# TorchIO-project/torchio

Hardware: AMD Instinct MI355X
Metric: volumes/s (256^3 float32) for Compose[affine+elastic+bias+blur+noise] (higher is better)
Workload: dtype f32; 1 GPU; Compose[Affine(+-10deg,0.9-1.1,+-5mm),ElasticDeformation(7^3cp,7.5mm),BiasField,Blur(0.5-2mm),Noise] on 1x256^3 f32, per-instance params; batch_per_gpu=8, global_batch=8, noise_rng=philox, resample_precision=tight, stencil_precision=fast, parallelism=batch-split x1 (no data-path collective)

## Files before the change

### torchio_amd/csrc/api.hip

```cpp
#include <stdarg.h>
#include <stdio.h>
#include <stdlib.h>
#include <string.h>

#include <atomic>
#include <mutex>

#include "common.hpp"

namespace tio {

static thread_local char g_error[512] = "";

void set_error(const char* fmt, ...) {
  va_list ap;
  va_start(ap, fmt);
  vsnprintf(g_error, sizeof(g_error), fmt, ap);
  va_end(ap);
}

int fail(int status, const char* fmt, ...) {
  va_list ap;
  va_start(ap, fmt);
  vsnprintf(g_error, sizeof(g_error), fmt, ap);
  va_end(ap);
  return status;
}

int check_launch(const char* what) {
  const hipError_t err = hipGetLastError();
  if (err != hipSuccess) return fail(TIO_ERR_LAUNCH, "%s: launch failed: %s", what, hipGetErrorString(err));
  return TIO_OK;
}

static std::atomic<const EnvSwitches*> g_env{nullptr};
static std::mutex g_env_mu;

static const EnvSwitches* parse_env() {
  EnvSwitches* e = new EnvSwitches();
  auto num = [](const char* name, int unset) { const char* v = getenv(name); return v != nullptr ? atoi(v) : unset; };
  e->nearest_kernel = num("TIO_NEAREST_KERNEL", 1) != 0;
  if (const char* v = getenv("TIO_NEAREST_EPS")) { e->has_nearest_eps = 1; e->nearest_eps = static_cast<float>(atof(v)); }
  if (const char* v = getenv("TIO_RESAMPLE_PATH")) e->resample_path = strcmp(v, "gather") == 0 ? 1 : (strcmp(v, "tile") == 0 ? 2 : 0);
  e->tile_variant = num("TIO_TILE_VARIANT", 0);
  e->tile_lds_floats = num("TIO_TILE_LDS_FLOATS", 0);
  e->tile_ablate = num("TIO_TILE_ABLATE", 0);
  e->resample_exact = getenv("TIO_RESAMPLE_EXACT") != nullptr;
  if (const char* v = getenv("TIO_FAST_KERNEL")) e->fast_kernel = strcmp(v, "brick") == 0 ? 1 : (strcmp(v, "planned") == 0 ? 2 : 0);
  e->planned_lean = num("TIO_PLANNED_LEAN", 1) != 0;
  e->dma_packed = num("TIO_DMA_PACKED", 1) != 0;
  e->exact_plan = num("TIO_EXACT_PLAN", -1);
  e->exact_lean = num("TIO_EXACT_LEAN", -1);
  e->lean_interleave = num("TIO_LEAN_INTERLEAVE", 1);
  e->lean_multi = num("TIO_LEAN_MULTI", 1);
  e->nearest_exact = num("TIO_NEAREST_EXACT", 1);
  e->lean_pair = num("TIO_LEAN_PAIR", 1);
  e->lean_label = num("TIO_LEAN_LABEL", 1);
  e->nearest_lds = num("TIO_NEAREST_LDS", -1);
  e->fast_fill_recheck = num("TIO_FAST_FILL_RECHECK", 1) != 0;
  e->conv_no_fuse = getenv("TIO_CONV_NO_FUSE") != nullptr;
  e->conv_ring = getenv("TIO_CONV_RING") != nullptr;
  e->march_segs = num("TIO_MARCH_SEGS", 0);
  e->march_order = num("TIO_MARCH_ORDER", -1);
  e->min_blocks = num("TIO_MIN_BLOCKS", 0);
  return e;
}

const EnvSwitches& env_switches() {
  const EnvSwitches* e = g_env.load(std::memory_order_acquire);
  if (e != nullptr) return *e;
  std::lock_guard<std::mutex> lock(g_env_mu);
  e = g_env.load(std::memory_order_acquire);
  if (e == nullptr) { e = parse_env(); g_env.store(e, std::memory_order_release); }
  return *e;
}

}

extern "C" void tio_reload_env(void) {
  std::lock_guard<std::mutex> lock(tio::g_env_mu);
  tio::g_env.store(tio::parse_env(), std::memory_order_release);
}

extern "C" int tio_abi_version(void) { return TIO_ABI_VERSION; }

extern "C" const char* tio_last_error(void) { return tio::g_error; }
// ... 10 lines not shown
```

### torchio_amd/csrc/common.hpp

```cpp
#pragma once

#include <hip/hip_runtime.h>
#include <stdint.h>

#include "../../include/tio_hip.h"

namespace tio {

void set_error(const char* fmt, ...);
int fail(int status, const char* fmt, ...);
int check_launch(const char* what);

struct EnvSwitches {
  int nearest_kernel = 1;
  int has_nearest_eps = 0;
  float nearest_eps = 0.0f;
  int resample_path = 0;
  int tile_variant = 0;
  int tile_lds_floats = 0;
  int tile_ablate = 0;
  int resample_exact = 0;
  int fast_kernel = 0;
  int planned_lean = 1;
  int dma_packed = 1;
  int exact_plan = -1;
  int exact_lean = -1;
  int nearest_exact = 1;
  int nearest_lds = -1;
  int lean_pair = 1;
  int lean_label = 1;
  int lean_multi = 1;
  int lean_interleave = 1;
  int fast_fill_recheck = 1;
  int conv_no_fuse = 0;
  int conv_ring = 0;
  int march_segs = 0;
  int march_order = -1;
  int min_blocks = 0;
};
const EnvSwitches& env_switches();

__device__ __forceinline__ float bf16_bits_to_float(uint16_t h) {
  return __uint_as_float(static_cast<uint32_t>(h) << 16);
}

__device__ __forceinline__ uint16_t float_to_bf16_bits(float f) {
  uint32_t x = __float_as_uint(f);
  if ((x & 0x7FFFFFFFu) > 0x7F800000u) return 0x7FC0u;
  x += 0x7FFFu + ((x >> 16) & 1u);
  return static_cast<uint16_t>(x >> 16);
}

template <int DT>
struct Elem;
template <>
struct Elem<TIO_F32> {
  using type = float;
  static __device__ __forceinline__ float load(const void* p, int64_t i) { return static_cast<const float*>(p)[i]; }
  static __device__ __forceinline__ void store(void* p, int64_t i, float v) { static_cast<float*>(p)[i] = v; }
};
template <>
struct Elem<TIO_F64> {
  using type = double;
  static __device__ __forceinline__ float load(const void* p, int64_t i) {
// ... 141 lines not shown
```

### torchio_amd/csrc/resample.hip

```cpp
#include <type_traits>
#include <stdlib.h>
#include <string.h>

#include <mutex>
#include <vector>
#include <algorithm>

#include "common.hpp"

namespace tio {

struct ImgArgs {
  const void* in;
  void* out;
  const float* fill;
  int channels;
  int dtype;
  int interp;
  const double* labels;
  int n_labels;
  double pad_label;
  float* out_min;
  uint32_t* min_keys;
};
// ... 780 lines not shown
    if (s.interp == TIO_LABEL_PV) {
      if (s.channels != 1)
        return fail(TIO_ERR_INVALID_ARGUMENT, "tio_resample3d: image %d: TIO_LABEL_PV needs channels == 1, got %d", i, s.channels);
      if (s.n_labels < 0 || (s.n_labels > 0 && s.labels_dev == nullptr))
        return fail(TIO_ERR_INVALID_ARGUMENT, "tio_resample3d: image %d: bad label table", i);
      pv.img[pv.n_images++] = ImgArgs{s.in, s.out, nullptr, 1, s.dtype, s.interp, s.labels_dev, s.n_labels, s.pad_label, nullptr, nullptr};
      continue;
    }
    if (nn_enabled && s.interp == TIO_NEAREST && s.out_min_dev == nullptr) {
      nn.img[nn.n_images++] = NearestImg{s.in, s.out, s.channels, dtype_size(s.dtype), s.fill_dev, s.dtype};
      if (s.fill_dev != nullptr) nn.any_fill = 1;
      continue;
    }
    a.img[a.n_images++] = ImgArgs{s.in, s.out, s.fill_dev, s.channels, s.dtype, s.interp, nullptr, 0, 0.0, s.out_min_dev, nullptr};
    if (s.interp == TIO_LINEAR || s.interp == TIO_LINEAR_ADJOINT || s.fill_dev != nullptr) a.any_linear = 1;
    if (s.interp == TIO_NEAREST) a.any_nearest = 1;
    const int need = s.dtype == TIO_F32 ? 0 : ((s.dtype == TIO_I16 || s.dtype == TIO_U8 || s.dtype == TIO_I32) ? 1 : 2);
    group.dtmode = need > group.dtmode ? need : group.dtmode;
    group.rows16 = group.rows16 && (reinterpret_cast<uintptr_t>(s.in) & 15) == 0;
  }
  return TIO_OK;
}

enum FloatRoadKind { kRoadGather, kRoadBrick, kRoadPlannedBrick, kRoadFastBrick, kRoadPlannedFast, kRoadPlannedLean, kRoadLeanExact };

struct FloatRoad {
  FloatRoadKind kind = kRoadGather;
  int variant = 0;
  bool exact_lerp = false;
  int64_t bricks = 0;
  size_t lds = 0;
  size_t plan_need = 0;
  int cp_lds = 0, tile_cap = 0, ablate = 0, fill_recheck = 0, dma_packed = 0, plan_multi = 0;
  int interleave = 0, pair = 0;
};
FloatRoad choose_float_road(const tio_resample_geom& geom, const ResampleArgs& a, const FloatGroup& g, const EnvSwitches& env) {
  FloatRoad r;
  bool use_tile = a.any_linear != 0;
  if (env.resample_path == 1) use_tile = false;
  if (env.resample_path == 2) use_tile = true;
  if (g.any_adjoint) use_tile = false;
  if (static_cast<int64_t>(a.Jo) * a.Ko * 8 >= (1LL << 31)) use_tile = false;
  if (static_cast<int64_t>(a.I) * a.J * a.K >= (1LL << 30)) use_tile = false;
  if (!use_tile) return r;
  r.kind = kRoadBrick;
  r.variant = env.tile_variant;
  r.ablate = env.tile_ablate;
  r.fill_recheck = env.fast_fill_recheck;
  r.cp_lds = control_points_fit_lds(a) ? ((control_floats(a) + 3) & ~3) : 0;
  const int bpc = r.variant == 3 ? 2 : ((r.variant == 2 || r.variant == 4) ? 4 : kTileBlocksPerCU);
  const int cap = env.tile_lds_floats > 0 ? env.tile_lds_floats : kLdsFloatsPerCU / bpc - 512 - r.cp_lds - kTileRedInts;
  const int max_cap = kLdsFloatsPerCU - r.cp_lds - kTileRedInts;
  r.tile_cap = cap < kTileMinCap ? kTileMinCap : (cap > max_cap ? max_cap : cap);
  r.lds = static_cast<size_t>(r.cp_lds + kTileRedInts + r.tile_cap) * sizeof(float);
  r.bricks = static_cast<int64_t>(a.B) * ((a.Io + 15) / 16) * ((a.Jo + 15) / 16) * ((a.Ko + 15) / 16);
  const size_t plan_plain = static_cast<size_t>(a.B) * 16 + static_cast<size_t>(r.bricks) * kDescInts;
  const bool fast = geom.precision == TIO_PRECISION_FAST && g.dtmode == 0 && !a.any_nearest && r.variant == 0 && !env.resample_exact;
  const bool tight = geom.precision == TIO_PRECISION_TIGHT && !env.resample_exact;
  const bool lean_exact = !fast && (tight || ((geom.precision == TIO_PRECISION_EXACT || geom.precision == TIO_PRECISION_TIGHT) && env.exact_lean != 0)) &&
                          g.dtmode == 0 && !a.any_nearest && r.variant == 0 && r.ablate == 0 && a.short_div != 0 && (a.cp == nullptr || a.unit_spacing != 0);
  if (fast || lean_exact) {
    const bool force_planned = lean_exact ? (env.fast_kernel == 2 || env.exact_lean == 2) : env.fast_kernel == 2;
    bool planned = (lean_exact || env.fast_kernel != 1) && (a.K & 3) == 0 && (r.bricks >= kPlannedMinBricks || force_planned) && r.bricks < (1LL << 26) && g.rows16;
    if ((geom.flags & (TIO_GEOM_LARGE_BOXES | TIO_GEOM_MOSTLY_LARGE_BOXES)) != 0 && !force_planned && !lean_exact) planned = false;
    if (planned && a.cp != nullptr) {
      const int n_ctl[3] = {a.ni, a.nj, a.nk}, n_vox[3] = {a.Io, a.Jo, a.Ko};
      for (int d = 0; d < 3; d++)
        if (n_ctl[d] > 2 && (n_vox[d] - 1) < 16 * (n_ctl[d] - 1)) planned = false;
    }
    if (planned) {
      r.kind = lean_exact ? kRoadLeanExact : (env.planned_lean != 0 ? kRoadPlannedLean : kRoadPlannedFast);
      r.exact_lerp = !tight;
      const int cap_p = env.tile_lds_floats > 0 ? env.tile_lds_floats : (kLdsFloatsPerCU / kTileBlocksPerCU) / 320 * 320;
      r.tile_cap = cap_p < kTileMinCap ? kTileMinCap : (cap_p > kLdsFloatsPerCU ? kLdsFloatsPerCU : cap_p);
      r.cp_lds = 0;
      r.lds = static_cast<size_t>(r.tile_cap) * sizeof(float);
      r.dma_packed = env.dma_packed;
      r.interleave = env.lean_interleave;
      r.pair = env.lean_pair;
      if (lean_exact && env.lean_multi != 0)
        r.plan_multi = (geom.flags & TIO_GEOM_MOSTLY_LARGE_BOXES) != 0 ? 2 : ((geom.flags & TIO_GEOM_LARGE_BOXES) != 0 ? 1 : 0);
      const size_t n = static_cast<size_t>(r.bricks);
      const size_t plan_multi_ints = static_cast<size_t>(a.B) * 16 + n * (kDescInts + kPassInts * kPassesPerBrick) + ((n + 3) & ~static_cast<size_t>(3));
      r.plan_need = (kPlanHeaderInts + (r.plan_multi ? plan_multi_ints : plan_plain)) * sizeof(int);
      return r;
    }
    if (fast) {
      r.kind = kRoadFastBrick;
      return r;
    }
  }
  if (r.variant == 0 && r.ablate == 0 && a.cp == nullptr && env.exact_plan != 0 && (r.bricks >= kPlannedMinBricks || env.exact_plan == 2) && r.bricks < (1LL << 26)) {
    r.kind = kRoadPlannedBrick;
    r.plan_need = (kPlanHeaderInts + plan_plain) * sizeof(int);
  }
  return r;
}

void apply_road(ResampleArgs& a, const FloatRoad& r) {
  a.fill_recheck = r.fill_recheck; a.ablate = r.ablate; a.cp_lds = r.cp_lds; a.tile_cap = r.tile_cap;
  a.dma_packed = r.dma_packed; a.plan_multi = r.plan_multi;
  for (int i = 0; i < a.n_images && r.kind != kRoadGather; i++) a.any_fill |= a.img[i].fill != nullptr ? 1 : 0;
}

LeanArgs make_lean_args(const ResampleArgs& a, const FloatRoad& r, const int* plan, int n_items) {
  LeanArgs la{};
  la.plan = plan; la.cp = a.cp;
  la.I = a.I; la.J = a.J; la.K = a.K; la.Io = a.Io; la.Jo = a.Jo; la.Ko = a.Ko;
  la.B = a.B; la.n_items = n_items;
  la.bricks_per_element = static_cast<unsigned>(a.tiles_i) * a.tiles_j * a.tiles_k;
  la.bpe_magic = magic_u32(la.bricks_per_element);
  la.ni = a.ni; la.nj = a.nj; la.nk = a.nk; la.cp_batched = a.cp_batched;
  la.sci = a.scale_i; la.scj = a.scale_j; la.sck = a.scale_k;
  for (int e = 0; e < 3; e++) la.dsc[e] = a.rsp[e] * (a.affine_first ? a.half_h[e] / a.dh[e] : 1.0f);
  la.hx = a.size_m1[0]; la.hy = a.size_m1[1]; la.hz = a.size_m1[2];
  la.affine_first = a.affine_first; la.ablate = a.ablate;
  la.mapping = a.mapping; la.mapping_batched = a.mapping_batched; la.unit_spacing = a.unit_spacing; la.fill_recheck = a.fill_recheck;
  for (int e = 0; e < 3; e++) { la.sp[e] = a.sp[e]; la.rsp[e] = a.rsp[e]; la.den[e] = a.den[e]; la.rden[e] = a.rden[e]; }
  for (int e = 0; e < 3; e++) { la.dh[e] = a.dh[e]; la.rdh[e] = a.rdh[e]; la.half_h[e] = a.half_h[e]; }
  la.interleave = r.interleave;
  la.tile_floats = r.tile_cap;
  return la;
}

struct LabelRide {
  int es = 0;
  unsigned blocks = 0, lds = 0;
};
void launch_nearest_exact(const NearestArgs& nn, int es, unsigned blocks, unsigned lds, hipStream_t s) {
  with_element_size(es, [&](auto size) {
    with_bools([&](auto elastic) { hipLaunchKernelGGL((resample_nearest_exact_kernel<elastic.value, size.value>), dim3(blocks), dim3(256), lds, s, nn); }, nn.cp != nullptr);
  });
}

int launch_nearest(NearestArgs& nn, bool short_div, bool floats_alone, const EnvSwitches& env, hipStream_t s, LabelRide* label) {
  const bool rows = nn.Ko >= 48;
  unsigned blocks = 0;
  if (const int st = set_tiles(nn, 16, rows ? 4 : 16, rows ? 64 : 16, &blocks)) return st;
  nn.eps = env.has_nearest_eps ? env.nearest_eps : kNearestEps;
  const bool exact = env.nearest_exact != 0 && nn.any_fill == 0 && rows && short_div && (nn.cp == nullptr || nn.unit_spacing != 0);
  const unsigned exact_lds = env.nearest_lds >= 0 ? static_cast<unsigned>(env.nearest_lds) : (nn.cp == nullptr ? 52000u : 0u);
  for (int es = 1; es <= 8; es *= 2) {
    bool present = false;
    for (int i = 0; i < nn.n_images; i++) present = present || nn.img[i].es == es;
    if (!present) continue;
    const int64_t n_in = static_cast<int64_t>(nn.I) * nn.J * nn.K, n_out = static_cast<int64_t>(nn.Io) * nn.Jo * nn.Ko;
    const bool narrow = static_cast<int64_t>(nn.I) * nn.J <= (1 << 24) && static_cast<int64_t>(nn.K) * es < (1 << 24) &&
                        n_in * es < (int64_t{1} << 32) - 16 && n_out * es < (int64_t{1} << 32) - 16;
    if (exact && narrow && env.lean_label != 0 && nn.n_images == 1 && nn.img[0].channels == 1 && es <= 4 && floats_alone) {
      label->es = es; label->blocks = blocks; label->lds = exact_lds;
    } else if (exact && narrow) {
      launch_nearest_exact(nn, es, blocks, exact_lds, s);
    } else {
// ... 257 lines not shown
```

### torchio_amd/csrc/resample_fast.hpp

```cpp
#pragma once

namespace tio {

typedef __attribute__((address_space(3))) const float* fast_lds_ptr;
typedef __attribute__((address_space(3))) float* fast_lds_wptr;

__device__ __forceinline__ void fast_axis(float src, int n, int& i0, int& i1, float& l) {
  const float c = fminf(fmaxf(floorf(src), 0.0f), static_cast<float>(n > 1 ? n - 2 : 0));
  i0 = static_cast<int>(c);
  i1 = min(i0 + 1, n - 1);
  l = fminf(fmaxf(src - c, 0.0f), 1.0f);
}

template <typename CP>
struct FastFrameT {
  float m[12];
  double c[3];
  int j_lo, k_lo;
  bool elastic, affine_first;
  CP cp;
  int ni, nj, nk;
  float sci, scj, sck;
  float dsc[3];
};
// ... 471 lines not shown
#pragma unroll
    for (int q = 0; q < 12; q++) {
      const float mv = m[q];
      weird |= (__float_as_uint(mv) & 0x7FFFFFFFu) > 0x7149F2CAu;
      f.m[q] = mv * ratio[q >> 2];
    }
  }
#pragma unroll
  for (int e = 0; e < 3; e++) f.dsc[e] = a.rsp[e] * (f.affine_first ? ratio[e] : 1.0f);
  if constexpr (ELASTIC_POSSIBLE) {
    f.elastic = !(a.cp_skip != nullptr && a.cp_skip[p.b] != 0);
    f.cp = f.elastic ? a.cp + (a.cp_batched ? static_cast<int64_t>(p.b) * (a.ni * a.nj * a.nk * 3) : 0) : nullptr;
  }
  pipe_brick_frame(f, p.j_lo, p.k_lo);
  int ext[7] = {-0x40000000, -0x40000000, -0x40000000, -0x40000000, -0x40000000, -0x40000000, 0};
  const int n_vert = f.elastic ? 27 : 8;
  if (v < n_vert) {
    int r[6]; bool bad;
    pipe_vertex(a, f, v, p.i_begin, p.i_count, p.nv, p.nw, r, bad);
#pragma unroll
    for (int q = 0; q < 6; q++) ext[q] = r[q];
    ext[6] = bad ? 1 : 0;
  }
#pragma unroll
  for (int s = GROUP / 2; s > 0; s >>= 1) {
#pragma unroll
    for (int q = 0; q < 7; q++) ext[q] = max(ext[q], __shfl_xor(ext[q], s));
  }
  const PlanBox whole = plan_box(a, ext, weird);
  const bool wrd = weird | (ext[6] != 0);
  int kind = whole.outside ? kDescOutside : (whole.fits ? kDescStaged : kDescSlow);
  PlanBox first = whole;
  int d15 = 0;
  if (a.plan_multi != 0 && kind == kDescSlow && !wrd) {
    int* passes = plan + a.B * 16 + n_items * kDescInts + t * (kPassInts * kPassesPerBrick);
    for (int nsplit = 2; nsplit <= 4; nsplit *= 2) {
      const int span = TI / nsplit;
      bool all_ok = true;
      for (int q = 0; q < nsplit; q++) {
        const int u0 = p.i_begin + q * span, n = min(span, p.i_begin + p.i_count - u0);
        int e7[7] = {-0x40000000, -0x40000000, -0x40000000, -0x40000000, -0x40000000, -0x40000000, 0};
        if (v < n_vert && n > 0) {
          int r[6]; bool bad;
          pipe_vertex(a, f, v, u0, n, p.nv, p.nw, r, bad);
#pragma unroll
          for (int c = 0; c < 6; c++) e7[c] = r[c];
          e7[6] = bad ? 1 : 0;
        }
#pragma unroll
        for (int sft = GROUP / 2; sft > 0; sft >>= 1) {
#pragma unroll
          for (int c = 0; c < 7; c++) e7[c] = max(e7[c], __shfl_xor(e7[c], sft));
        }
        PlanBox pb = plan_pass_box(a, e7, weird);
        if (n <= 0) { pb.outside = 1; pb.fits = 0; pb.interior = 0; }
        all_ok &= (pb.fits | pb.outside) != 0;
        const int state = pb.outside ? kPassOutside : (pb.fits ? kPassStaged : kPassSlow);
        if (q == 0) { first = pb; d15 = nsplit; }
        d15 |= state << (8 + 4 * q);
        if (v == 0) {
          int* r8 = passes + q * kPassInts;
          r8[0] = pb.xmin; r8[1] = pb.ymin; r8[2] = pb.za; r8[3] = pb.Lx; r8[4] = pb.Ly; r8[5] = pb.cpr;
          r8[6] = state | (pb.interior << 8); r8[7] = max(n, 0);
        }
      }
      kind = kDescMulti;
// ... 181 lines not shown
        first = false;
      }
      float A3[3], B3[3];
      int run0 = u0;
      int run1 = fast_column_line(f, lj, lk, planes, run0, u1, u0, C3, col3, lane, A3, B3);
      tile_dma_wait();
      __syncthreads();
      const bool track = g.out_min != nullptr && b == 0;
      uint32_t kmin = 0xFFFFFFFFu;
      unsigned unsure = 0u;
      const float margin = (a.fill_recheck != 0 && has_fill) ? ((const_float_ptr)(plan) + b * 16)[12] : -1.0f;
      if (col_active) {
        for (;;) {
          char* o_run = out_chan + static_cast<int64_t>(run0) * slab_b;
          if (track)
            fast_sample_line<4, true>(run1 - run0, A3, B3, ta, o_run, urow, slab_b, has_fill & !bx.interior, ox, oy, oz, hx, hy, hz, fillv, kmin, margin, run0 - u0, unsure);
          else
            fast_sample_line<4, false>(run1 - run0, A3, B3, ta, o_run, urow, slab_b, has_fill & !bx.interior, ox, oy, oz, hx, hy, hz, fillv, kmin, margin, run0 - u0, unsure);
          run0 = run1;
          if (run0 >= u1) break;
          run1 = fast_column_line(f, lj, lk, planes, run0, u1, u0, C3, col3, lane, A3, B3);
        }
      }
      if (has_fill & !bx.interior)
        fast_fill_tail<ELASTIC_POSSIBLE>(unsure, a, a.mapping + (a.mapping_batched ? b * 12 : 0), elastic, f.cp, lj, lk, u0, static_cast<float>(j_lo + jv),
                                         static_cast<float>(k_lo + kw), in_chan, a.I, a.J, a.K, hx, hy, hz, fillv, out_chan, slab_b, urow, track ? &kmin : nullptr);
      if (track) publish_min(g, c, kmin);
    }
  }
}



struct LeanArgs {
  const float* in;
  float* out;
  int64_t in_stride, out_stride;
  const float* fill;
  const int* plan;
  const float* cp;
  int I, J, K, Io, Jo, Ko;
  int B, n_items;
  unsigned bricks_per_element, bpe_magic;
  int ni, nj, nk, cp_batched;
  float sci, scj, sck;
  float dsc[3];
  float hx, hy, hz;
  int affine_first, ablate;
  const float* mapping;
  int mapping_batched, unit_spacing, fill_recheck;
  float sp[3], rsp[3], den[3], rden[3];
  float dh[3], rdh[3], half_h[3];
  int interleave;
  int tile_floats;
  int last_use;
  uint32_t* min_keys;
  const float* in2;
  float* out2;
  int64_t in_stride2, out_stride2;
  const float* fill2;
  const void* lab_in;
  void* lab_out;
  int lab_es;
};

__device__ __forceinline__ float lean_gather(const float* __restrict__ chan, int I, int J, int K, float x, float y, float z, bool has_fill,
// ... 221 lines not shown
```

### torchio_amd/csrc/resample_lean_exact.hpp

```cpp
#pragma once

namespace tio {

__device__ __forceinline__ void tile_dma_wait_all() { asm volatile("s_waitcnt vmcnt(0) lgkmcnt(0)" ::: "memory"); }

template <int NW>
struct BoxDmaStepper {
  typedef __attribute__((address_space(1))) const char* global_byte_ptr;
  global_byte_ptr origin;
  float* lp;
  unsigned off, step_b, wrap_b;
  int row, p, r;
  int step, step_p, step_r, total_rows, Ly, lp_step;
  int bx0, by0, I, J;
  int left;
  bool ch_ok, lane_ok;

  __device__ __forceinline__ void init(float* tile, const float* src, const StreamBox& bx, int I_, int J_, int K, int wave, int lane) {
    StageLanes sl;
    sl.cpr = -1; sl.rpi = 1; sl.row_l = 0; sl.gz_rel = 0; sl.goff = 0; sl.lane_ok = false;
    stage_lanes(sl, bx.cpr, K, lane);
    const int rpi = sl.rpi;
    total_rows = bx.Lx * bx.Ly;
    const int n_instr = __builtin_amdgcn_readfirstlane(static_cast<int>((static_cast<float>(total_rows + rpi - 1) + 0.5f) * __builtin_amdgcn_rcpf(static_cast<float>(rpi))));
    step = NW * rpi;
    const float rcp_ly = __builtin_amdgcn_rcpf(static_cast<float>(bx.Ly));
    step_p = __builtin_amdgcn_readfirstlane(static_cast<int>((static_cast<float>(step) + 0.5f) * rcp_ly));
    step_r = step - step_p * bx.Ly;
    row = wave * rpi + sl.row_l;
    p = static_cast<int>((static_cast<float>(row) + 0.5f) * rcp_ly);
    r = row - p * bx.Ly;
    const unsigned plane_b = static_cast<unsigned>(J_) * static_cast<unsigned>(K) * 4u, row_b = static_cast<unsigned>(K) * 4u;
    off = static_cast<unsigned>(p) * plane_b + static_cast<unsigned>(r) * row_b + static_cast<unsigned>(sl.gz_rel) * 4u;
    step_b = static_cast<unsigned>(step_p) * plane_b + static_cast<unsigned>(step_r) * row_b;
    wrap_b = plane_b - static_cast<unsigned>(bx.Ly) * row_b;
    origin = (global_byte_ptr)(src) + ((static_cast<int64_t>(bx.bx0) * J_ + bx.by0) * K + bx.za) * 4;
    const int dgroup = rpi * bx.cpr * 4;
    lp = tile + wave * dgroup;
    lp_step = NW * dgroup;
    ch_ok = static_cast<unsigned>(bx.za + sl.gz_rel) < static_cast<unsigned>(K);
    lane_ok = sl.lane_ok;
    Ly = bx.Ly; bx0 = bx.bx0; by0 = bx.by0; I = I_; J = J_;
    left = n_instr > wave ? (n_instr - wave + NW - 1) / NW : 0;
  }

  template <bool INTERIOR>
  __device__ __forceinline__ void issue(int lane) {
    const bool in_box = lane_ok & (row < total_rows);
    if constexpr (INTERIOR) {
      if (in_box) __builtin_amdgcn_global_load_lds(origin + off, (fast_lds_wptr)(lp), 16, 0, 0);
    } else {
      const bool in_vol = in_box & ch_ok & (static_cast<unsigned>(bx0 + p) < static_cast<unsigned>(I)) &
                          (static_cast<unsigned>(by0 + r) < static_cast<unsigned>(J));
      if (in_vol) __builtin_amdgcn_global_load_lds(origin + off, (fast_lds_wptr)(lp), 16, 0, 0);
      else if (in_box) {
        lds_zero_chunk(lp + 4 * lane);
      }
    }
    row += step; p += step_p; r += step_r; off += step_b;
    if (r >= Ly) { r -= Ly; p += 1; off += wrap_b; }
    lp += lp_step;
    left -= 1;
  }
};

template <int MODE, bool UNIT, bool SHORT>
__device__ __forceinline__ void lean_exact_coord(const float (&m)[12], const LeanArgs& a, float ci, float cj, float ck, float di, float dj,
                                                 float dk, float& x, float& y, float& z) {
#define TIO_LE_ROW(R, A, B, C) \
  __builtin_fmaf(1.0f, m[4 * R + 3], __builtin_fmaf(C, m[4 * R + 2], __builtin_fmaf(B, m[4 * R + 1], __fmul_rn(A, m[4 * R]))))
  float vi, vj, vk;
  if constexpr (MODE == 0) {
    vi = TIO_LE_ROW(0, ci, cj, ck); vj = TIO_LE_ROW(1, ci, cj, ck); vk = TIO_LE_ROW(2, ci, cj, ck);
  } else {
    float qi = di, qj = dj, qk = dk;
    if constexpr (!UNIT) {
// ... 127 lines not shown
  const bool by0 = (y0 >= 0.0f) & (y0 <= hy), by1 = (y1 >= 0.0f) & (y1 <= hy);
  const bool bz0 = (z0 >= 0.0f) & (z0 <= hz), bz1 = (z1 >= 0.0f) & (z1 <= hz);
  const int ix0 = static_cast<int>(fminf(fmaxf(x0, 0.0f), hx)), ix1 = static_cast<int>(fminf(fmaxf(x1, 0.0f), hx));
  const int iy0 = static_cast<int>(fminf(fmaxf(y0, 0.0f), hy)), iy1 = static_cast<int>(fminf(fmaxf(y1, 0.0f), hy));
  const int iz0 = static_cast<int>(fminf(fmaxf(z0, 0.0f), hz)), iz1 = static_cast<int>(fminf(fmaxf(z1, 0.0f), hz));
  float val = 0.0f, mask = 0.0f;
#pragma unroll
  for (int k = 0; k < 8; k++) {
    const float w = __fmul_rn(__fmul_rn((k & 1) ? wx1 : wx0, (k & 2) ? wy1 : wy0), (k & 4) ? wz1 : wz0);
    const bool ok = ((k & 1) ? bx1 : bx0) & ((k & 2) ? by1 : by0) & ((k & 4) ? bz1 : bz0);
    const int off = (((k & 1) ? ix1 : ix0) * J + ((k & 2) ? iy1 : iy0)) * K + ((k & 4) ? iz1 : iz0);
    const float v = chan[off];
    const float next_v = __fadd_rn(val, __fmul_rn(v, w));
    const float next_m = __fadd_rn(mask, w);
    val = ok ? next_v : val;
    mask = ok ? next_m : mask;
  }
  if (has_fill) val = (mask > 0.5f) ? val : fillv;
  return val;
}

template <bool EXACT_LERP, bool MASKED>
__device__ __forceinline__ void lean_exact_group_values(const float (&X4)[4], const float (&Y4)[4], const float (&Z4)[4], const TileAddr& ta, float hx,
                                                        float hy, float hz, bool has_fill, float fillv, float (&vals)[4]) {
  TapSet ts[4];
#pragma unroll
  for (int u = 0; u < 4; u++) tile_issue_folded(ts[u], X4[u], Y4[u], Z4[u], ta);
  __builtin_amdgcn_sched_barrier(0);
#pragma unroll
  for (int u = 0; u < 4; u++) {
    float val = EXACT_LERP ? tile_finish(ts[u]) : tile_finish_fast(ts[u]);
    if constexpr (MASKED) val = (!has_fill || tile_mask(ts[u], X4[u], Y4[u], Z4[u], hx, hy, hz) > 0.5f) ? val : fillv;
    vals[u] = val;
  }
}

template <bool GUARD, bool TRACK>
__device__ __forceinline__ void lean_exact_group_store(const float (&vals)[4], char*& out_generic, unsigned urow, int64_t slab_b, int t0, int i_count,
                                                       bool col_active, uint32_t& kmin) {
  typedef __attribute__((address_space(1))) char* global_char_ptr;
  typedef __attribute__((address_space(1))) float* global_float_ptr;
  global_char_ptr out_t = (global_char_ptr)out_generic;
  unsigned row_off = urow;
  asm volatile("" : "+v"(row_off));
#pragma unroll
  for (int u = 0; u < 4; u++) {
    const bool live = !GUARD || (col_active && (t0 + u) < i_count);
    if (live) {
      *(global_float_ptr)(out_t + row_off) = vals[u];
      if constexpr (TRACK) kmin = min(kmin, float_to_key(vals[u]));
    }
    out_t += slab_b;
    asm volatile("" : "+s"(out_t));
  }
  out_generic = (char*)out_t;
}

template <bool EXACT_LERP, bool MASKED, bool GUARD, bool TRACK>
__device__ __forceinline__ void lean_exact_group(const float (&X4)[4], const float (&Y4)[4], const float (&Z4)[4], const TileAddr& ta, char*& out_generic,
                                                 unsigned urow, int64_t slab_b, int t0, int i_count, bool col_active, float hx, float hy,
                                                 float hz, bool has_fill, float fillv, uint32_t& kmin) {
  float vals[4];
  lean_exact_group_values<EXACT_LERP, MASKED>(X4, Y4, Z4, ta, hx, hy, hz, has_fill, fillv, vals);
  lean_exact_group_store<GUARD, TRACK>(vals, out_generic, urow, slab_b, t0, i_count, col_active, kmin);
  __builtin_amdgcn_sched_barrier(0);
}
// ... 164 lines not shown
  if (ka->ablate & 512) return;
  if (es == 1) TIO_LE_LABEL_STORES(uint8_t)
  else if (es == 2) TIO_LE_LABEL_STORES(uint16_t)
  else TIO_LE_LABEL_STORES(uint32_t)
#undef TIO_LE_LABEL_STORES
}

template <bool ELASTIC_POSSIBLE, bool EXACT_LERP, bool FOLD_MIN, bool MULTI, bool PAIR = false, bool LABEL = false>
__device__ __forceinline__ void lean_exact_brick(const LeanArgs& a, const unsigned brick, float* s_tile) {
  static_assert(!PAIR || (!FOLD_MIN && !MULTI), "the pair kernel has no folded minimum and no passes");
  static_assert(!LABEL || (!FOLD_MIN && !MULTI), "a label channel rides along launches without a folded minimum and without passes");
  constexpr int TI = 16, TJ = 16, TK = 16, NW = 4;
  typedef __attribute__((address_space(4))) const int* const_int_ptr;
  typedef __attribute__((address_space(4))) const float* const_float_ptr;

  {
    const int* plan_p = a.plan; const float* in_p = a.in; const float* map_p = a.mapping; float* out_p = a.out; const float* fill_p = a.fill;
    asm volatile("" ::"s"(a.n_items), "s"(a.bricks_per_element), "s"(a.bpe_magic), "s"(plan_p), "s"(in_p), "s"(map_p), "s"(a.B), "s"(a.I), "s"(a.J), "s"(a.K),
                 "s"(a.mapping_batched), "s"(a.tile_floats), "s"(a.in_stride), "s"(a.out_stride), "s"(a.Io), "s"(a.Jo), "s"(a.Ko), "s"(a.interleave),
                 "s"(out_p), "s"(fill_p), "s"(a.hx), "s"(a.hy), "s"(a.hz), "s"(a.affine_first));
    if constexpr (ELASTIC_POSSIBLE) {
      const float* cp_p = a.cp;
      asm volatile("" ::"s"(cp_p), "s"(a.cp_batched), "s"(a.ni), "s"(a.nj), "s"(a.nk), "s"(a.sci), "s"(a.scj), "s"(a.sck));
    }
  }
  const int b = static_cast<int>(fastdiv_exact(brick, a.bpe_magic, a.bricks_per_element));
  const_int_ptr d = (const_int_ptr)(a.plan + a.B * 16) + static_cast<size_t>(brick) * kDescInts;
  const_float_ptr mp = (const_float_ptr)(a.mapping) + (a.mapping_batched ? b * 12 : 0);
  const int kind_w = d[0];
  StreamBox bx;
  bx.bx0 = d[1]; bx.by0 = d[2]; bx.za = d[3]; bx.Lx = d[4]; bx.Ly = d[5]; bx.cpr = d[6];
  const int i_begin = d[11], j_lo = d[12], k_lo = d[13];
  const int elastic_w = d[14];
  int multi_w = 0, plan_tile = 0;
  if constexpr (MULTI) {
    multi_w = d[15];
    plan_tile = ((const_int_ptr)(a.plan))[b * 16 + 13];
  }
  float m[12];
#pragma unroll
  for (int q = 0; q < 12; q++) m[q] = mp[q];
  asm volatile("" ::"s"(kind_w), "s"(i_begin), "s"(j_lo), "s"(k_lo), "s"(elastic_w));
  if constexpr (MULTI) asm volatile("" ::"s"(multi_w), "s"(plan_tile));
  const bool elastic = ELASTIC_POSSIBLE && elastic_w != 0;

  const int tid = threadIdx.x;
  const int lane = tid & 63;
  const int wave = __builtin_amdgcn_readfirstlane(tid >> 6);
  const int tk = tid & (TK - 1), tj = tid / TK;
  const int slab = a.Jo * a.Ko;
  const int64_t slab_b = static_cast<int64_t>(slab) * 4;
  const float* in_chan = a.in + static_cast<int64_t>(b) * a.in_stride;
  char* out_chan = reinterpret_cast<char*>(a.out + static_cast<int64_t>(b) * a.out_stride);

  int kind = kind_w & 0xFF;
  const bool multi = MULTI && kind == kDescMulti;
  if constexpr (!MULTI) {
    if (kind == kDescMulti) return;
  }
  int nsplit = 1, states = 0;
  if constexpr (MULTI) {
    if (multi) {
      nsplit = multi_w & 0xF; states = multi_w >> 8;
      kind = plan_tile <= a.tile_floats ? kDescStaged : kDescSlow;
    }
  }
  if (!multi && kind == kDescStaged && (static_cast<int64_t>(bx.Lx) * bx.Ly * (bx.cpr * 4) > static_cast<int64_t>(a.tile_floats) ||
                                        !box_address_fits(bx.bx0, bx.by0, bx.za, bx.Lx, bx.Ly, bx.cpr)))
    kind = kDescSlow;
  if (kind == kDescSlow) states = 0x2222;
  const int span_shift = nsplit == 4 ? 2 : (nsplit == 2 ? 3 : 4);
  bx.kind = kind; bx.interior = kind_w >> 8;
  BoxDmaStepper<NW> dma;
  dma.left = 0;
  if (kind == kDescStaged && (states & 0xF) == kPassStaged) dma.init(s_tile, in_chan, bx, a.I, a.J, a.K, wave, lane);

  const int i_count = min(TI, a.Io - i_begin), nv = min(TJ, a.Jo - j_lo), nw = min(TK, a.Ko - k_lo);
  const bool col_active = (tj < nv) & (tk < nw);
  const bool full = (i_count == TI) & (nv == TJ) & (nw == TK);
  const int jv = min(tj, nv - 1), kw = min(tk, nw - 1);
  const int col_off = (j_lo + jv) * a.Ko + (k_lo + kw);
  const unsigned urow = static_cast<unsigned>(col_off) * 4u;
  bool has_fill = a.fill != nullptr;
  float fillv = has_fill ? ((const_float_ptr)a.fill)[0] : 0.0f;
  const float hx = a.hx, hy = a.hy, hz = a.hz;

  const bool track = FOLD_MIN && a.min_keys != nullptr && b == 0;
  uint32_t kmin = 0xFFFFFFFFu;
  auto publish_min = [&]() {
    const uint32_t wmin = wave_min_u32(kmin);
    if (lane == 0 && wmin != 0xFFFFFFFFu)
      __hip_atomic_fetch_min(a.min_keys + (brick & (kMinSlots - 1)), wmin, __ATOMIC_RELAXED, __HIP_MEMORY_SCOPE_AGENT);
  };
  if (kind == kDescGated || kind == kDescOutside) {
    if (col_active) {
      for (int t = i_begin; t < i_begin + i_count; t++) {
        const float val = kind == kDescGated ? in_chan[static_cast<int64_t>(t) * slab + col_off] : fillv;
        *reinterpret_cast<float*>(out_chan + t * slab_b + urow) = val;
        kmin = min(kmin, float_to_key(val));
      }
    }
    if constexpr (LABEL) {
      if (col_active) {
        const int es = a.lab_es;
        const int64_t n_out_l = static_cast<int64_t>(a.Io) * slab;
        for (int t = i_begin; t < i_begin + i_count; t++) {
          const int64_t e = b * n_out_l + static_cast<int64_t>(t) * slab + col_off;
          lean_label_store(a.lab_out, es, e, kind == kDescGated ? lean_label_load(a.lab_in, es, e) : 0u);
        }
      }
    }
    if constexpr (PAIR) {
// ... 11 lines not shown

  const float cj = static_cast<float>(j_lo + jv), ck = static_cast<float>(k_lo + kw);
  const float* cp = elastic ? a.cp + (a.cp_batched ? static_cast<int64_t>(b) * (a.ni * a.nj * a.nk * 3) : 0) : nullptr;
  Lerp1D lj{0, 0, 1.0f, 0.0f}, lk{0, 0, 1.0f, 0.0f};
  if constexpr (ELASTIC_POSSIBLE) {
    if (elastic) {
      lj = lerp_index(j_lo + jv, a.nj, a.Jo, a.scj);
      lk = lerp_index(k_lo + kw, a.nk, a.Ko, a.sck);
    }
  }
  const int i_last = i_begin + i_count - 1;
  Lerp1D li_lane{0, 0, 1.0f, 0.0f};
  int ia = 0, ib = 0;
  if constexpr (ELASTIC_POSSIBLE) {
    if (elastic) {
      li_lane = lerp_index(min(i_begin + (lane & (TI - 1)), i_last), a.ni, a.Io, a.sci);
      ia = __builtin_amdgcn_readlane(li_lane.i0, 0);
      ib = __builtin_amdgcn_readlane(li_lane.i1, TI - 1);
    }
  }

  if (elastic && ib - ia > 2) states = 0x2222;
  bool any_staged = states == 0;
  if constexpr (MULTI) {
    for (int pass = 0; pass < nsplit; pass++) any_staged |= ((states >> (4 * pass)) & 0xF) == kPassStaged;
  }
  if (!any_staged) {
    lean_exact_slow_planes<ELASTIC_POSSIBLE, false, LABEL>(brick, states, span_shift, kmin);
    if constexpr (PAIR) lean_exact_slow_planes<ELASTIC_POSSIBLE, true>(brick, states, span_shift, kmin);
    if (track) publish_min();
    return;
  }

  if (a.interleave == 2 && bx.interior) {
    while (dma.left > 0) dma.template issue<true>(lane);
  }
  CtlPlanes P{0.f, 0.f, 0.f, 0.f, 0.f, 0.f, 0.f, 0.f, 0.f};
  if constexpr (ELASTIC_POSSIBLE) {
    if (elastic) {
      const int s_i = a.nj * a.nk * 3, s_j = a.nk * 3;
      float pa[3], pb[3], pc[3];
      cp_plane(cp, ia, s_i, s_j, lj, lk, pa);
      cp_plane(cp, min(ia + 1, a.ni - 1), s_i, s_j, lj, lk, pb);
      cp_plane(cp, min(ia + 2, a.ni - 1), s_i, s_j, lj, lk, pc);
      P.a_i = pa[0]; P.a_j = pa[1]; P.a_k = pa[2];
      P.b_i = pb[0]; P.b_j = pb[1]; P.b_k = pb[2];
      P.c_i = pc[0]; P.c_j = pc[1]; P.c_k = pc[2];
      asm volatile("" : "+v"(P.a_i), "+v"(P.a_j), "+v"(P.a_k), "+v"(P.b_i), "+v"(P.b_j), "+v"(P.b_k), "+v"(P.c_i), "+v"(P.c_j), "+v"(P.c_k));
    }
  }
  if (!bx.interior) {
    while (dma.left > 0) dma.template issue<false>(lane);
  }
  if (!a.interleave) {
    while (dma.left > 0) dma.template issue<true>(lane);
  }
  float X[TI], Y[TI], Z[TI];
  const bool ident = (m[0] == 1.0f) & (m[1] == 0.0f) & (m[2] == 0.0f) & (m[3] == 0.0f) & (m[4] == 0.0f) & (m[5] == 1.0f) &
                     (m[6] == 0.0f) & (m[7] == 0.0f) & (m[8] == 0.0f) & (m[9] == 0.0f) & (m[10] == 1.0f) & (m[11] == 0.0f);
  bool done = false;
  if constexpr (ELASTIC_POSSIBLE) {
    if (elastic) {
      if (ident) lean_exact_planes<1, true, true, true, NW>(m, a, i_begin, i_last, cj, ck, li_lane, ia, P, dma, lane, X, Y, Z);
      else if (a.affine_first) lean_exact_planes<2, true, true, true, NW>(m, a, i_begin, i_last, cj, ck, li_lane, ia, P, dma, lane, X, Y, Z);
      else lean_exact_planes<3, true, true, true, NW>(m, a, i_begin, i_last, cj, ck, li_lane, ia, P, dma, lane, X, Y, Z);
      done = true;
    }
  }
  if (!done) lean_exact_planes<0, true, true, true, NW>(m, a, i_begin, i_last, cj, ck, li_lane, ia, P, dma, lane, X, Y, Z);
  while (dma.left > 0) dma.template issue<true>(lane);

  TileAddr ta;
  auto set_tile_addr = [&](const StreamBox& box) {
    ta.ox = static_cast<float>(box.bx0); ta.oy = static_cast<float>(box.by0); ta.oz = static_cast<float>(box.za);
    ta.sYb = box.cpr * 16; ta.sXb = box.Ly * ta.sYb; ta.sXYb = ta.sXb + ta.sYb;
    ta.sYbf = static_cast<float>(ta.sYb); ta.sXbf = static_cast<float>(ta.sXb);
    ta.base_f = static_cast<float>(static_cast<unsigned>(reinterpret_cast<uintptr_t>((fast_lds_wptr)s_tile)));
    ta.c_f = ta.base_f - ta.ox * ta.sXbf - ta.oy * ta.sYbf - 4.0f * ta.oz;
  };
  set_tile_addr(bx);

  unsigned vlab[16];
  (void)vlab;
  if constexpr (LABEL) {
    lean_exact_label_issue(X, Y, Z, b, vlab);
    tile_dma_wait_keep16();
  } else {
    tile_dma_wait_all();
  }
  __syncthreads();

  char* out_t = out_chan + static_cast<int64_t>(i_begin) * slab_b;
  bool may_leave = has_fill & !bx.interior;
  if constexpr (!MULTI) {
#define TIO_LE_COORDS4                                                          \
  const float x4[4] = {X[4 * q], X[4 * q + 1], X[4 * q + 2], X[4 * q + 3]};     \
  const float y4[4] = {Y[4 * q], Y[4 * q + 1], Y[4 * q + 2], Y[4 * q + 3]};     \
  const float z4[4] = {Z[4 * q], Z[4 * q + 1], Z[4 * q + 2], Z[4 * q + 3]};
#define TIO_LE_GROUPS(TRACK)                                                                                                              \
  _Pragma("unroll") for (int q = 0; q < 4; q++) {                                                                                         \
    TIO_LE_COORDS4                                                                                                                        \
    bool masked = false;                                                                                                                  \
    if (may_leave) masked = __builtin_amdgcn_ballot_w64(lean_exact_group_leaves(x4, y4, z4, hx, hy, hz)) != 0ull;                         \
    if (masked)                                                                                                                           \
      lean_exact_group<EXACT_LERP, true, false, TRACK>(x4, y4, z4, ta, out_t, urow, slab_b, 4 * q, i_count, col_active, hx, hy, hz, true, fillv, kmin);   \
    else                                                                                                                                  \
      lean_exact_group<EXACT_LERP, false, false, TRACK>(x4, y4, z4, ta, out_t, urow, slab_b, 4 * q, i_count, col_active, hx, hy, hz, false, fillv, kmin); \
  }
#define TIO_LE_GROUPS_GUARDED(TRACK)                                                                                                      \
  _Pragma("unroll") for (int q = 0; q < 4; q++) {                                                                                         \
    TIO_LE_COORDS4                                                                                                                        \
    lean_exact_group<EXACT_LERP, true, true, TRACK>(x4, y4, z4, ta, out_t, urow, slab_b, 4 * q, i_count, col_active, hx, hy, hz, has_fill, fillv, kmin); \
  }
    if constexpr (PAIR) {
      if (full) { TIO_LE_GROUPS(false) } else { TIO_LE_GROUPS_GUARDED(false) }
      __syncthreads();
      typedef __attribute__((address_space(4))) const LeanArgs* const_args_ptr;
      const_args_ptr ka = (const_args_ptr)__builtin_amdgcn_kernarg_segment_ptr();
      asm volatile("" : "+s"(ka));
      const_int_ptr d2 = (const_int_ptr)(ka->plan + ka->B * 16) + static_cast<size_t>(brick) * kDescInts;
      StreamBox nb;
      nb.bx0 = d2[1]; nb.by0 = d2[2]; nb.za = d2[3]; nb.Lx = d2[4]; nb.Ly = d2[5]; nb.cpr = d2[6];
      nb.interior = d2[0] >> 8; nb.kind = kDescStaged;
      BoxDmaStepper<NW> step;
      step.init(s_tile, ka->in2 + static_cast<int64_t>(b) * ka->in_stride2, nb, ka->I, ka->J, ka->K, wave, lane);
// ... 133 lines not shown
```

Before: 6080 volumes/s.

## Stage tile DMA wait so early output planes compute while later planes load

The planner now computes, for interior staged boxes, how many leading input planes the first half of the output rows actually need, and stores that count in the descriptor. The lean exact kernel waits only for the DMA instructions that cover those lead planes, barriers, computes the first eight voxels from LDS, then waits for the rest before finishing. The goal is to overlap global-to-LDS staging latency with interpolation work. The cost is extra planner work (vertex evaluation plus shuffles), an added barrier, and register pressure from holding the early values. Correctness depends on the vmcnt-based partial wait matching the DMA issue order.

```diff
diff --git a/torchio_amd/csrc/api.hip b/torchio_amd/csrc/api.hip
--- a/torchio_amd/csrc/api.hip
+++ b/torchio_amd/csrc/api.hip
@@ -52,6 +52,7 @@
   e->exact_plan = num("TIO_EXACT_PLAN", -1);
   e->exact_lean = num("TIO_EXACT_LEAN", -1);
   e->lean_interleave = num("TIO_LEAN_INTERLEAVE", 1);
+  e->lean_staged_wait = num("TIO_LEAN_STAGED_WAIT", 1);
   e->lean_multi = num("TIO_LEAN_MULTI", 1);
   e->nearest_exact = num("TIO_NEAREST_EXACT", 1);
   e->lean_pair = num("TIO_LEAN_PAIR", 1);
diff --git a/torchio_amd/csrc/common.hpp b/torchio_amd/csrc/common.hpp
--- a/torchio_amd/csrc/common.hpp
+++ b/torchio_amd/csrc/common.hpp
@@ -30,6 +30,7 @@
   int lean_pair = 1;
   int lean_label = 1;
   int lean_multi = 1;
+  int lean_staged_wait = 1;
   int lean_interleave = 1;
   int fast_fill_recheck = 1;
   int conv_no_fuse = 0;
diff --git a/torchio_amd/csrc/resample.hip b/torchio_amd/csrc/resample.hip
--- a/torchio_amd/csrc/resample.hip
+++ b/torchio_amd/csrc/resample.hip
@@ -836,7 +836,7 @@
   size_t lds = 0;
   size_t plan_need = 0;
   int cp_lds = 0, tile_cap = 0, ablate = 0, fill_recheck = 0, dma_packed = 0, plan_multi = 0;
-  int interleave = 0, pair = 0;
+  int interleave = 0, pair = 0, staged_wait = 0;
 };
 FloatRoad choose_float_road(const tio_resample_geom& geom, const ResampleArgs& a, const FloatGroup& g, const EnvSwitches& env) {
   FloatRoad r;
@@ -882,6 +882,7 @@
       r.dma_packed = env.dma_packed;
       r.interleave = env.lean_interleave;
       r.pair = env.lean_pair;
+      r.staged_wait = env.lean_staged_wait;
       if (lean_exact && env.lean_multi != 0)
         r.plan_multi = (geom.flags & TIO_GEOM_MOSTLY_LARGE_BOXES) != 0 ? 2 : ((geom.flags & TIO_GEOM_LARGE_BOXES) != 0 ? 1 : 0);
       const size_t n = static_cast<size_t>(r.bricks);
@@ -922,7 +923,7 @@
   la.mapping = a.mapping; la.mapping_batched = a.mapping_batched; la.unit_spacing = a.unit_spacing; la.fill_recheck = a.fill_recheck;
   for (int e = 0; e < 3; e++) { la.sp[e] = a.sp[e]; la.rsp[e] = a.rsp[e]; la.den[e] = a.den[e]; la.rden[e] = a.rden[e]; }
   for (int e = 0; e < 3; e++) { la.dh[e] = a.dh[e]; la.rdh[e] = a.rdh[e]; la.half_h[e] = a.half_h[e]; }
-  la.interleave = r.interleave;
+  la.interleave = (r.interleave & 3) | (r.staged_wait != 0 ? 0 : kLeanSingleWait);
   la.tile_floats = r.tile_cap;
   return la;
 }
diff --git a/torchio_amd/csrc/resample_fast.hpp b/torchio_amd/csrc/resample_fast.hpp
--- a/torchio_amd/csrc/resample_fast.hpp
+++ b/torchio_amd/csrc/resample_fast.hpp
@@ -527,6 +527,25 @@
   int kind = whole.outside ? kDescOutside : (whole.fits ? kDescStaged : kDescSlow);
   PlanBox first = whole;
   int d15 = 0;
+  if (kind == kDescStaged) {
+    d15 = whole.Lx;
+    if (whole.interior && !wrd && p.i_count > TI / 2) {
+      int e7[7] = {-0x40000000, -0x40000000, -0x40000000, -0x40000000, -0x40000000, -0x40000000, 0};
+      if (v < n_vert) {
+        int r[6]; bool bad;
+        pipe_vertex(a, f, v, p.i_begin, TI / 2, p.nv, p.nw, r, bad);
+#pragma unroll
+        for (int c = 0; c < 6; c++) e7[c] = r[c];
+        e7[6] = bad ? 1 : 0;
+      }
+#pragma unroll
+      for (int sft = GROUP / 2; sft > 0; sft >>= 1) {
+#pragma unroll
+        for (int c = 0; c < 7; c++) e7[c] = max(e7[c], __shfl_xor(e7[c], sft));
+      }
+      if (e7[6] == 0 && -e7[0] == whole.xmin) d15 = min(max(e7[1] + 2 - whole.xmin, 1), whole.Lx);
+    }
+  }
   if (a.plan_multi != 0 && kind == kDescSlow && !wrd) {
     int* passes = plan + a.B * 16 + n_items * kDescInts + t * (kPassInts * kPassesPerBrick);
     for (int nsplit = 2; nsplit <= 4; nsplit *= 2) {
@@ -774,6 +793,7 @@
 
 
 
+enum : int { kLeanSingleWait = 4 };
 struct LeanArgs {
   const float* in;
   float* out;
diff --git a/torchio_amd/csrc/resample_lean_exact.hpp b/torchio_amd/csrc/resample_lean_exact.hpp
--- a/torchio_amd/csrc/resample_lean_exact.hpp
+++ b/torchio_amd/csrc/resample_lean_exact.hpp
@@ -14,15 +14,18 @@
   int step, step_p, step_r, total_rows, Ly, lp_step;
   int bx0, by0, I, J;
   int left;
+  int late;
   bool ch_ok, lane_ok;
 
-  __device__ __forceinline__ void init(float* tile, const float* src, const StreamBox& bx, int I_, int J_, int K, int wave, int lane) {
+  __device__ __forceinline__ void init(float* tile, const float* src, const StreamBox& bx, int I_, int J_, int K, int wave, int lane, int lead_planes = 0) {
     StageLanes sl;
     sl.cpr = -1; sl.rpi = 1; sl.row_l = 0; sl.gz_rel = 0; sl.goff = 0; sl.lane_ok = false;
     stage_lanes(sl, bx.cpr, K, lane);
     const int rpi = sl.rpi;
     total_rows = bx.Lx * bx.Ly;
-    const int n_instr = __builtin_amdgcn_readfirstlane(static_cast<int>((static_cast<float>(total_rows + rpi - 1) + 0.5f) * __builtin_amdgcn_rcpf(static_cast<float>(rpi))));
+    const float rcp_rpi = __builtin_amdgcn_rcpf(static_cast<float>(rpi));
+    const int n_instr = __builtin_amdgcn_readfirstlane(static_cast<int>((static_cast<float>(total_rows + rpi - 1) + 0.5f) * rcp_rpi));
+    const int n_lead = __builtin_amdgcn_readfirstlane(static_cast<int>((static_cast<float>(lead_planes * bx.Ly + rpi - 1) + 0.5f) * rcp_rpi));
     step = NW * rpi;
     const float rcp_ly = __builtin_amdgcn_rcpf(static_cast<float>(bx.Ly));
     step_p = __builtin_amdgcn_readfirstlane(static_cast<int>((static_cast<float>(step) + 0.5f) * rcp_ly));
@@ -42,6 +45,7 @@
     lane_ok = sl.lane_ok;
     Ly = bx.Ly; bx0 = bx.bx0; by0 = bx.by0; I = I_; J = J_;
     left = n_instr > wave ? (n_instr - wave + NW - 1) / NW : 0;
+    late = left - (n_lead > wave ? (n_lead - wave + NW - 1) / NW : 0);
   }
 
   template <bool INTERIOR>
@@ -235,6 +239,64 @@
     float val = EXACT_LERP ? tile_finish(ts[u]) : tile_finish_fast(ts[u]);
     if constexpr (MASKED) val = (!has_fill || tile_mask(ts[u], X4[u], Y4[u], Z4[u], hx, hy, hz) > 0.5f) ? val : fillv;
     vals[u] = val;
+  }
+}
+
+typedef float lean_pair_t __attribute__((ext_vector_type(2)));
+__device__ __forceinline__ void lean_exact_taps_issue(TapSet& ts, lean_pair_t (&pr)[4], float x, float y, float z, const TileAddr& ta) {
+  const float x0 = floorf(x), y0 = floorf(y), z0 = floorf(z);
+  const float x1 = x0 + 1.0f, y1 = y0 + 1.0f, z1 = z0 + 1.0f;
+  ts.wx0 = x1 - x; ts.wx1 = x - x0; ts.wy0 = y1 - y; ts.wy1 = y - y0; ts.wz0 = z1 - z; ts.wz1 = z - z0;
+  const float af = __builtin_fmaf(x0, ta.sXbf, __builtin_fmaf(y0, ta.sYbf, __builtin_fmaf(z0, 4.0f, ta.c_f)));
+  const unsigned addr = static_cast<unsigned>(static_cast<int>(af));
+  const unsigned a10 = addr + ta.sXb, a01 = addr + ta.sYb, a11 = addr + ta.sXYb;
+  asm volatile("ds_read2_b32 %0, %1 offset1:1" : "=v"(pr[0]) : "v"(addr));
+  asm volatile("ds_read2_b32 %0, %1 offset1:1" : "=v"(pr[1]) : "v"(a10));
+  asm volatile("ds_read2_b32 %0, %1 offset1:1" : "=v"(pr[2]) : "v"(a01));
+  asm volatile("ds_read2_b32 %0, %1 offset1:1" : "=v"(pr[3]) : "v"(a11));
+}
+template <int U>
+__device__ __forceinline__ void lean_exact_taps_wait(TapSet& ts, lean_pair_t (&pr)[4]) {
+  static_assert(U >= 0 && U < 4, "four voxels per group");
+  if constexpr (U == 0) asm volatile("s_waitcnt lgkmcnt(12)" : "+v"(pr[0]), "+v"(pr[1]), "+v"(pr[2]), "+v"(pr[3]));
+  else if constexpr (U == 1) asm volatile("s_waitcnt lgkmcnt(8)" : "+v"(pr[0]), "+v"(pr[1]), "+v"(pr[2]), "+v"(pr[3]));
+  else if constexpr (U == 2) asm volatile("s_waitcnt lgkmcnt(4)" : "+v"(pr[0]), "+v"(pr[1]), "+v"(pr[2]), "+v"(pr[3]));
+  else asm volatile("s_waitcnt lgkmcnt(0)" : "+v"(pr[0]), "+v"(pr[1]), "+v"(pr[2]), "+v"(pr[3]));
+  ts.v[0] = pr[0].x; ts.v[4] = pr[0].y;
+  ts.v[1] = pr[1].x; ts.v[5] = pr[1].y;
+  ts.v[2] = pr[2].x; ts.v[6] = pr[2].y;
+  ts.v[3] = pr[3].x; ts.v[7] = pr[3].y;
+}
+template <bool EXACT_LERP>
+__device__ __forceinline__ void lean_exact_group_values_early(const float (&X4)[4], const float (&Y4)[4], const float (&Z4)[4], const TileAddr& ta,
+                                                              float (&vals)[4]) {
+  TapSet ts[4];
+  lean_pair_t pr[4][4];
+#pragma unroll
+  for (int u = 0; u < 4; u++) lean_exact_taps_issue(ts[u], pr[u], X4[u], Y4[u], Z4[u], ta);
+  __builtin_amdgcn_sched_barrier(0);
+  lean_exact_taps_wait<0>(ts[0], pr[0]);
+  vals[0] = EXACT_LERP ? tile_finish(ts[0]) : tile_finish_fast(ts[0]);
+  __builtin_amdgcn_sched_barrier(0);
+  lean_exact_taps_wait<1>(ts[1], pr[1]);
+  vals[1] = EXACT_LERP ? tile_finish(ts[1]) : tile_finish_fast(ts[1]);
+  __builtin_amdgcn_sched_barrier(0);
+  lean_exact_taps_wait<2>(ts[2], pr[2]);
+  vals[2] = EXACT_LERP ? tile_finish(ts[2]) : tile_finish_fast(ts[2]);
+  __builtin_amdgcn_sched_barrier(0);
+  lean_exact_taps_wait<3>(ts[3], pr[3]);
+  vals[3] = EXACT_LERP ? tile_finish(ts[3]) : tile_finish_fast(ts[3]);
+  __builtin_amdgcn_sched_barrier(0);
+}
+__device__ __forceinline__ void tile_dma_wait_keep(int late) {
+  switch (min(late, 6)) {
+    case 6: asm volatile("s_waitcnt vmcnt(6) lgkmcnt(0)" ::: "memory"); break;
+    case 5: asm volatile("s_waitcnt vmcnt(5) lgkmcnt(0)" ::: "memory"); break;
+    case 4: asm volatile("s_waitcnt vmcnt(4) lgkmcnt(0)" ::: "memory"); break;
+    case 3: asm volatile("s_waitcnt vmcnt(3) lgkmcnt(0)" ::: "memory"); break;
+    case 2: asm volatile("s_waitcnt vmcnt(2) lgkmcnt(0)" ::: "memory"); break;
+    case 1: asm volatile("s_waitcnt vmcnt(1) lgkmcnt(0)" ::: "memory"); break;
+    default: asm volatile("s_waitcnt vmcnt(0) lgkmcnt(0)" ::: "memory"); break;
   }
 }
 
@@ -465,6 +527,9 @@
   bx.bx0 = d[1]; bx.by0 = d[2]; bx.za = d[3]; bx.Lx = d[4]; bx.Ly = d[5]; bx.cpr = d[6];
   const int i_begin = d[11], j_lo = d[12], k_lo = d[13];
   const int elastic_w = d[14];
+  constexpr bool STAGES = !MULTI && !PAIR && !LABEL;
+  int lead_w = 0;
+  if constexpr (STAGES) lead_w = d[15];
   int multi_w = 0, plan_tile = 0;
   if constexpr (MULTI) {
     multi_w = d[15];
@@ -506,11 +571,16 @@
   bx.kind = kind; bx.interior = kind_w >> 8;
   BoxDmaStepper<NW> dma;
   dma.left = 0;
-  if (kind == kDescStaged && (states & 0xF) == kPassStaged) dma.init(s_tile, in_chan, bx, a.I, a.J, a.K, wave, lane);
+  dma.late = 0;
+  if (kind == kDescStaged && (states & 0xF) == kPassStaged) dma.init(s_tile, in_chan, bx, a.I, a.J, a.K, wave, lane, lead_w);
 
   const int i_count = min(TI, a.Io - i_begin), nv = min(TJ, a.Jo - j_lo), nw = min(TK, a.Ko - k_lo);
   const bool col_active = (tj < nv) & (tk < nw);
   const bool full = (i_count == TI) & (nv == TJ) & (nw == TK);
+  int stage_late = -1;
+  if constexpr (STAGES) {
+    if ((a.interleave & kLeanSingleWait) == 0 && kind == kDescStaged && bx.interior != 0 && full && lead_w >= 1 && lead_w < bx.Lx) stage_late = dma.late;
+  }
   const int jv = min(tj, nv - 1), kw = min(tk, nw - 1);
   const int col_off = (j_lo + jv) * a.Ko + (k_lo + kw);
   const unsigned urow = static_cast<unsigned>(col_off) * 4u;
@@ -588,7 +658,7 @@
     return;
   }
 
-  if (a.interleave == 2 && bx.interior) {
+  if ((a.interleave & 3) == 2 && bx.interior) {
     while (dma.left > 0) dma.template issue<true>(lane);
   }
   CtlPlanes P{0.f, 0.f, 0.f, 0.f, 0.f, 0.f, 0.f, 0.f, 0.f};
@@ -608,7 +678,7 @@
   if (!bx.interior) {
     while (dma.left > 0) dma.template issue<false>(lane);
   }
-  if (!a.interleave) {
+  if ((a.interleave & 3) == 0) {
     while (dma.left > 0) dma.template issue<true>(lane);
   }
   float X[TI], Y[TI], Z[TI];
@@ -636,6 +706,50 @@
   };
   set_tile_addr(bx);
 
+  char* out_t = out_chan + static_cast<int64_t>(i_begin) * slab_b;
+  if constexpr (STAGES) {
+    if (stage_late >= 0) {
+      tile_dma_wait_keep(stage_late);
+      __builtin_amdgcn_s_barrier();
+      __builtin_amdgcn_sched_barrier(0);
+      float v0[4], v1[4];
+      {
+        const float x4[4] = {X[0], X[1], X[2], X[3]}, y4[4] = {Y[0], Y[1], Y[2], Y[3]}, z4[4] = {Z[0], Z[1], Z[2], Z[3]};
+        lean_exact_group_values_early<EXACT_LERP>(x4, y4, z4, ta, v0);
+      }
+      {
+        const float x4[4] = {X[4], X[5], X[6], X[7]}, y4[4] = {Y[4], Y[5], Y[6], Y[7]}, z4[4] = {Z[4], Z[5], Z[6], Z[7]};
+        lean_exact_group_values_early<EXACT_LERP>(x4, y4, z4, ta, v1);
+      }
+      __builtin_amdgcn_s_waitcnt(0x0070);
+      __builtin_amdgcn_s_barrier();
+      __builtin_amdgcn_sched_barrier(0);
+      if (FOLD_MIN && track) {
+        lean_exact_group_store<false, true>(v0, out_t, urow, slab_b, 0, i_count, col_active, kmin);
+        lean_exact_group_store<false, true>(v1, out_t, urow, slab_b, 4, i_count, col_active, kmin);
+        __builtin_amdgcn_sched_barrier(0);
+#pragma unroll
+        for (int q = 2; q < 4; q++) {
+          const float x4[4] = {X[4 * q], X[4 * q + 1], X[4 * q + 2], X[4 * q + 3]}, y4[4] = {Y[4 * q], Y[4 * q + 1], Y[4 * q + 2], Y[4 * q + 3]};
+          const float z4[4] = {Z[4 * q], Z[4 * q + 1], Z[4 * q + 2], Z[4 * q + 3]};
+          lean_exact_group<EXACT_LERP, false, false, true>(x4, y4, z4, ta, out_t, urow, slab_b, 4 * q, i_count, col_active, hx, hy, hz, false, fillv, kmin);
+        }
+        publish_min();
+      } else {
+        lean_exact_group_store<false, false>(v0, out_t, urow, slab_b, 0, i_count, col_active, kmin);
+        lean_exact_group_store<false, false>(v1, out_t, urow, slab_b, 4, i_count, col_active, kmin);
+        __builtin_amdgcn_sched_barrier(0);
+#pragma unroll
+        for (int q = 2; q < 4; q++) {
+          const float x4[4] = {X[4 * q], X[4 * q + 1], X[4 * q + 2], X[4 * q + 3]}, y4[4] = {Y[4 * q], Y[4 * q + 1], Y[4 * q + 2], Y[4 * q + 3]};
+          const float z4[4] = {Z[4 * q], Z[4 * q + 1], Z[4 * q + 2], Z[4 * q + 3]};
+          lean_exact_group<EXACT_LERP, false, false, false>(x4, y4, z4, ta, out_t, urow, slab_b, 4 * q, i_count, col_active, hx, hy, hz, false, fillv, kmin);
+        }
+      }
+      return;
+    }
+  }
+
   unsigned vlab[16];
   (void)vlab;
   if constexpr (LABEL) {
@@ -646,7 +760,6 @@
   }
   __syncthreads();
 
-  char* out_t = out_chan + static_cast<int64_t>(i_begin) * slab_b;
   bool may_leave = has_fill & !bx.interior;
   if constexpr (!MULTI) {
 #define TIO_LE_COORDS4                                                          \
```

Result: no change. 6061 volumes/s (-0.3%).
